# EffortlessMetrics/BitNet-rs

Measured on AMD Instinct MI355X. Metric: decode tokens/sec + I2_S matmul HBM GB/s (% roofline), bitnet-b1.58-2B-4T, higher is better.
Workload: dtype i8 MFMA on producer-quantised activations (QAct: 15-bit fixed point per element, one power-of-two scale per 16), exact integer partial sums, f32 accumulate / f32 elsewhere (f16 embedding table); 1 GPU; bitnet-b1.58-2B-4T I2_S BitNet32-F16 (ternary, one f16 scale per 32 weights), 1xMI355X, batch=1 decode, 128-token prompt; layers=30, prompt_len=128, parallelism=single GPU, launch=hipGraph replay per token, kv_cache=f32 (as the reference, T:1171-1202)

## Files before the change

bitnet-rs_amd/csrc/kernels_decode.hip:

```cpp
#include <cstdlib>

#include "common.hpp"

namespace bitnet_hip {

typedef _Float16 half8 __attribute__((ext_vector_type(8)));

__device__ __forceinline__ float wsum(float v) {
#pragma unroll
    for (int off = 32; off > 0; off >>= 1) v += __shfl_xor(v, off, 64);
    return v;
}
__device__ __forceinline__ float wmax(float v) {
#pragma unroll
    for (int off = 32; off > 0; off >>= 1) v = fmaxf(v, __shfl_xor(v, off, 64));
    return v;
}
__device__ __forceinline__ float bsum(float v, float *slot) {
    v = wsum(v);
    __syncthreads();
    if ((threadIdx.x & 63) == 0) slot[threadIdx.x >> 6] = v;
    __syncthreads();
    return (slot[0] + slot[1]) + (slot[2] + slot[3]);
}
__device__ __forceinline__ float bmax(float v, float *slot) {
    v = wmax(v);
    __syncthreads();
    if ((threadIdx.x & 63) == 0) slot[threadIdx.x >> 6] = v;
    __syncthreads();
    return fmaxf(fmaxf(slot[0], slot[1]), fmaxf(slot[2], slot[3]));
}

__global__ void k_embed_f16(const _Float16 *__restrict__ table, const int *__restrict__ tokens,
                            const int *__restrict__ offset_ptr, int n, int hidden, int vocab,
                            float *__restrict__ out) {
    const int per_row = hidden >> 3;
    const int gid = blockIdx.x * blockDim.x + threadIdx.x;
    if (gid >= n * per_row) return;
    const int t = gid / per_row, c = gid % per_row;
    int tok = tokens[t + (offset_ptr ? *offset_ptr : 0)];
    tok = tok < 0 ? 0 : (tok >= vocab ? vocab - 1 : tok);
    const half8 h = *reinterpret_cast<const half8 *>(table + (size_t)tok * hidden + 8 * c);
    float *o = out + (size_t)t * hidden + 8 * c;
#pragma unroll
    for (int i = 0; i < 8; ++i) o[i] = (float)h[i];
}

hipError_t launch_embed_f16(const void *table, const int *tokens, const int *offset_ptr, int n, int hidden,
                            int vocab, float *out, hipStream_t stream) {
    const int total = n * (hidden >> 3);
    hipLaunchKernelGGL(k_embed_f16, dim3((total + 255) / 256), dim3(256), 0, stream,
                       static_cast<const _Float16 *>(table), tokens, offset_ptr, n, hidden, vocab, out);
    return hipGetLastError();
}

template <bool RMS>
__global__ __launch_bounds__(256) void k_norm_rows(const float *__restrict__ x, const float *__restrict__ gamma,
                                                   float *__restrict__ out, int hidden, float eps) {
    __shared__ float slot[4];
    const float *xr = x + (size_t)blockIdx.x * hidden;
    float *orow = out + (size_t)blockIdx.x * hidden;
    float mean = 0.0f;
    if (!RMS) {
        float s = 0.0f;
        for (int i = threadIdx.x; i < hidden; i += 256) s += xr[i];
        mean = bsum(s, slot) / (float)hidden;
    }
    float ss = 0.0f;
    for (int i = threadIdx.x; i < hidden; i += 256) {
        const float d = xr[i] - mean;
        ss += d * d;
    }
    const float denom = sqrtf(bsum(ss, slot) / (float)hidden + eps);
    for (int i = threadIdx.x; i < hidden; i += 256) orow[i] = (xr[i] - mean) / denom * gamma[i];
}

hipError_t launch_norm_rows(const float *x, const float *gamma, float *out, int rows, int hidden, float eps,
                            bool rms, hipStream_t stream) {
    if (rows <= 0) return hipSuccess;
    if (rms)
        hipLaunchKernelGGL(k_norm_rows<true>, dim3(rows), dim3(256), 0, stream, x, gamma, out, hidden, eps);
    else
        hipLaunchKernelGGL(k_norm_rows<false>, dim3(rows), dim3(256), 0, stream, x, gamma, out, hidden, eps);
    return hipGetLastError();
}

constexpr int kLogitChunks = 16;

template <int NCH, int R, bool GUARD = false>
__global__ __launch_bounds__(256) void k_logits_f16(const _Float16 *__restrict__ table, const float *__restrict__ x,
                                                    const float *__restrict__ gamma, float eps, int hidden, int vocab,
                                                    float *__restrict__ logits, float *__restrict__ best_val,
                                                    int *__restrict__ best_idx) {
    extern __shared__ __attribute__((aligned(16))) float xs[];
    __shared__ float slot[4];
    __shared__ float wbv[4];
    __shared__ int wbi[4];
    const int tid = threadIdx.x, lane = tid & 63, wave = tid >> 6;
    float s = 0.0f;
    for (int i = tid; i < hidden; i += 256) s += x[i];
    const float mean = gamma ? bsum(s, slot) / (float)hidden : 0.0f;
    float ss = 0.0f;
    for (int i = tid; i < hidden; i += 256) {
        const float d = x[i] - mean;
        ss += d * d;
    }
    const float denom = gamma ? sqrtf(bsum(ss, slot) / (float)hidden + eps) : 1.0f;
    for (int i = tid; i < hidden; i += 256) xs[i] = gamma ? (x[i] - mean) / denom * gamma[i] : x[i];
    __syncthreads();
    const int nchunks = hidden >> 9;
    float xr[NCH][8];
#pragma unroll
    for (int c = 0; c < NCH; ++c)
#pragma unroll
        for (int i = 0; i < 8; ++i) xr[c][i] = (!GUARD || c < nchunks) ? xs[512 * c + 8 * lane + i] : 0.0f;
    float bv = -INFINITY;
    int bi = 0x7fffffff;
    const int total_waves = gridDim.x * 4;
    for (int row = (blockIdx.x * 4 + wave) * R; row < vocab; row += total_waves * R) {
        half8 w[R][NCH];
#pragma unroll
        for (int r = 0; r < R; ++r) {
            const _Float16 *e = table + (size_t)(row + r < vocab ? row + r : vocab - 1) * hidden + 8 * lane;
#pragma unroll
            for (int c = 0; c < NCH; ++c)
                w[r][c] = __builtin_nontemporal_load(reinterpret_cast<const half8 *>(e + 512 * ((!GUARD || c < nchunks) ? c : 0)));
        }
        float acc[R];
#pragma unroll
        for (int r = 0; r < R; ++r) {
            acc[r] = 0.0f;
#pragma unroll
            for (int c = 0; c < NCH; ++c)
#pragma unroll
                for (int i = 0; i < 8; ++i) acc[r] += xr[c][i] * (float)w[r][c][i];
        }
#pragma unroll
        for (int off = 32; off > 0; off >>= 1)
#pragma unroll
            for (int r = 0; r < R; ++r) acc[r] += __shfl_xor(acc[r], off, 64);
        if (lane == 0) {
#pragma unroll
            for (int r = 0; r < R; ++r)
                if (row + r < vocab) {
                    logits[row + r] = acc[r];
                    const float v = acc[r] != acc[r] ? -INFINITY : acc[r];
                    if (v > bv || (v == bv && row + r < bi)) {
                        bv = v;
                        bi = row + r;
                    }
                }
        }
    }
    if (lane == 0) {
        wbv[wave] = bv;
        wbi[wave] = bi;
    }
    __syncthreads();
    if (tid == 0) {
        for (int w2 = 1; w2 < 4; ++w2)
            if (wbv[w2] > bv || (wbv[w2] == bv && wbi[w2] < bi)) {
                bv = wbv[w2];
                bi = wbi[w2];
            }
        best_val[blockIdx.x] = bv;
        best_idx[blockIdx.x] = bi;
    }
}

__global__ __launch_bounds__(256) void k_argmax_final(const float *__restrict__ best_val, const int *__restrict__ best_idx,
                                                      int n, int *__restrict__ token_out, int *__restrict__ pos_ptr,
                                                      int *__restrict__ history, const int *__restrict__ n_forced) {
    __shared__ float sv[256];
    __shared__ int si[256];
    float bv = -INFINITY;
    int bi = 0x7fffffff;
    for (int i = threadIdx.x; i < n; i += 256) {
        const float v = best_val[i];
        const int idx = best_idx[i];
        if (v > bv || (v == bv && idx < bi)) {
            bv = v;
            bi = idx;
        }
    }
    sv[threadIdx.x] = bv;
    si[threadIdx.x] = bi;
    __syncthreads();
    for (int off = 128; off > 0; off >>= 1) {
        if ((int)threadIdx.x < off) {
            const float v = sv[threadIdx.x + off];
            const int idx = si[threadIdx.x + off];
            if (v > sv[threadIdx.x] || (v == sv[threadIdx.x] && idx < si[threadIdx.x])) {
                sv[threadIdx.x] = v;
                si[threadIdx.x] = idx;
            }
        }
        __syncthreads();
    }
    if (threadIdx.x == 0) {
        const int tok = si[0] == 0x7fffffff ? 0 : si[0];
        if (token_out) *token_out = tok;
        if (pos_ptr) {
            const int p = *pos_ptr;
            if (history && (!n_forced || p + 1 >= *n_forced)) history[p + 1] = tok;
            *pos_ptr = p + 1;
        }
    }
}

hipError_t launch_logits_f16(const void *table, const float *x, const float *gamma, float eps, int hidden, int vocab,
                             float *logits, float *best_val, int *best_idx, int n_wg, hipStream_t stream) {
    if (hidden % 512 != 0 || hidden > 512 * kLogitChunks) return hipErrorInvalidValue;
    void (*kfn)(const _Float16 *, const float *, const float *, float, int, int, float *, float *, int *) = nullptr;
    static const int rows = getenv("BITNET_HIP_LOGIT_ROWS") ? atoi(getenv("BITNET_HIP_LOGIT_ROWS")) : 3;
    switch (hidden / 512) {
        case 1: kfn = k_logits_f16<1, 4>; break;
        case 2: kfn = k_logits_f16<2, 4>; break;
        case 4: kfn = k_logits_f16<4, 4>; break;
        case 5: kfn = rows == 2 ? k_logits_f16<5, 2> : rows == 3 ? k_logits_f16<5, 3> : k_logits_f16<5, 4>; break;
        case 8: kfn = k_logits_f16<8, 2>; break;
        default: kfn = hidden / 512 <= 8 ? k_logits_f16<8, 2, true> : k_logits_f16<16, 1, true>; break;
    }
    hipLaunchKernelGGL(kfn, dim3(n_wg), dim3(256), (size_t)hidden * sizeof(float), stream, static_cast<const _Float16 *>(table), x, gamma,
                       eps, hidden, vocab, logits, best_val, best_idx);
    return hipGetLastError();
}

hipError_t launch_argmax_final(const float *best_val, const int *best_idx, int n, int *token_out, int *pos_ptr,
                               int *history, const int *n_forced, hipStream_t stream) {
    hipLaunchKernelGGL(k_argmax_final, dim3(1), dim3(256), 0, stream, best_val, best_idx, n, token_out, pos_ptr, history,
                       n_forced);
    return hipGetLastError();
}

__global__ void k_add(const float *__restrict__ a, const float *__restrict__ b, float *__restrict__ out, size_t n) {
    const size_t i = (size_t)blockIdx.x * blockDim.x + threadIdx.x;
    if (i < n) out[i] = a[i] + b[i];
}
hipError_t launch_add(const float *a, const float *b, float *out, size_t n, hipStream_t stream) {
    hipLaunchKernelGGL(k_add, dim3((unsigned)((n + 255) / 256)), dim3(256), 0, stream, a, b, out, n);
    return hipGetLastError();
}
__global__ void k_silu_mul(const float *__restrict__ gate, const float *__restrict__ up, float *__restrict__ out, size_t n, size_t tile) {
    const size_t i = (size_t)blockIdx.x * blockDim.x + threadIdx.x;
    if (i >= n) return;
    const size_t j = tile ? (i / tile) * 2 * tile + i % tile : i;
    const float g = gate[j], u = up[j];
    out[i] = g / (1.0f + expf(-g)) * u;
}
hipError_t launch_silu_mul(const float *gate, const float *up, float *out, size_t n, size_t tile, hipStream_t stream) {
    hipLaunchKernelGGL(k_silu_mul, dim3((unsigned)((n + 255) / 256)), dim3(256), 0, stream, gate, up, out, n, tile);
    return hipGetLastError();
}

__global__ void k_advance_pos(int *pos_ptr) {
    if (threadIdx.x == 0 && blockIdx.x == 0) *pos_ptr = *pos_ptr + 1;
}
hipError_t launch_advance_pos(int *pos_ptr, hipStream_t stream) {
    hipLaunchKernelGGL(k_advance_pos, dim3(1), dim3(64), 0, stream, pos_ptr);
    return hipGetLastError();
}

__global__ __launch_bounds__(256) void k_argmax_partial(const float *__restrict__ v, int n, float *__restrict__ best_val,
                                                        int *__restrict__ best_idx) {
    __shared__ float sv[256];
    __shared__ int si[256];
    float bv = -INFINITY;
    int bi = 0x7fffffff;
    for (int i = blockIdx.x * 256 + threadIdx.x; i < n; i += gridDim.x * 256) {
        const float a = v[i] != v[i] ? -INFINITY : v[i];
        if (a > bv || (a == bv && i < bi)) {
            bv = a;
            bi = i;
        }
    }
    sv[threadIdx.x] = bv;
    si[threadIdx.x] = bi;
    __syncthreads();
    for (int off = 128; off > 0; off >>= 1) {
        if ((int)threadIdx.x < off) {
            const float a = sv[threadIdx.x + off];
            const int idx = si[threadIdx.x + off];
            if (a > sv[threadIdx.x] || (a == sv[threadIdx.x] && idx < si[threadIdx.x])) {
                sv[threadIdx.x] = a;
                si[threadIdx.x] = idx;
            }
        }
        __syncthreads();
    }
    if (threadIdx.x == 0) {
        best_val[blockIdx.x] = sv[0];
        best_idx[blockIdx.x] = si[0];
    }
}

hipError_t launch_argmax(const float *v, int n, float *best_val, int *best_idx, int n_wg, int *token_out,
                         hipStream_t stream) {
    hipLaunchKernelGGL(k_argmax_partial, dim3(n_wg), dim3(256), 0, stream, v, n, best_val, best_idx);
    hipLaunchKernelGGL(k_argmax_final, dim3(1), dim3(256), 0, stream, best_val, best_idx, n_wg, token_out, nullptr, nullptr, nullptr);
    return hipGetLastError();
}

__global__ __launch_bounds__(512) void k_stream_read(const uint4 *__restrict__ buf, size_t n_vec, unsigned *sink) {
    const size_t stride = (size_t)gridDim.x * 512 * 8;
    unsigned acc = 0;
    for (size_t i = ((size_t)blockIdx.x * 8) * 512 + threadIdx.x; i < n_vec; i += stride) {
        uint4 v[8];
#pragma unroll
        for (int j = 0; j < 8; ++j) {
            const size_t idx = i + (size_t)j * 512;
            const unsigned *p = reinterpret_cast<const unsigned *>(buf + (idx < n_vec ? idx : i));
            v[j].x = __builtin_nontemporal_load(p);
            v[j].y = __builtin_nontemporal_load(p + 1);
            v[j].z = __builtin_nontemporal_load(p + 2);
            v[j].w = __builtin_nontemporal_load(p + 3);
        }
#pragma unroll
        for (int j = 0; j < 8; ++j) acc ^= v[j].x ^ v[j].y ^ v[j].z ^ v[j].w;
    }
    if (acc == 0x9e3779b9u) *sink = acc;
}

hipError_t launch_stream_read(const void *buf, size_t bytes, unsigned *sink, hipStream_t stream) {
    const size_t n_vec = bytes / 16;
    size_t grid = div_ceil(n_vec, (size_t)512 * 8 * 4);
    if (grid < 256) grid = 256;
    if (grid > 65535u * 16u) grid = 65535u * 16u;
    hipLaunchKernelGGL(k_stream_read, dim3((unsigned)grid), dim3(512), 0, stream, static_cast<const uint4 *>(buf), n_vec, sink);
    return hipGetLastError();
}

}
```

bitnet-rs_amd/host/decoder.hpp:

```cpp
#pragma once

#include <cstddef>
#include <cstdint>
#include <string>
#include <vector>

#include "bitnet_hip.h"

extern "C" {
typedef int (*bitnet_host_allgather_fn)(void *ctx, const void *send_dev, void *recv_dev, size_t bytes_per_rank, void *stream);
}

namespace bitnet_host {

struct Config {
    int hidden = 2560, n_layers = 30, n_heads = 20, n_kv_heads = 5, head_dim = 128;
    int ffn = 6912, vocab = 128256, max_pos = 4096;
    float eps = 1e-5f;
    float rope_theta = 10000.f;
};

struct LayerWeightsQk256 {
    const float *attn_norm, *ffn_norm;
    const uint8_t *q, *k, *v, *o, *gate, *up, *down;
};
struct LayerWeightsI2s {
    const float *attn_norm, *ffn_norm;
    const uint8_t *w[7];
    const float *scales[7];
    size_t block_size;
};

struct ProjSpec {
    bool qk256 = true;
    const uint8_t *bytes = nullptr;
    size_t len = 0;
    const float *scales = nullptr;
    size_t n_scales = 0, block = 32;
    int8_t code_map[4] = {-2, -1, 0, 1};
};

class Decoder {
  public:
    explicit Decoder(const Config &cfg);
    ~Decoder();
    Decoder(const Decoder &) = delete;
    Decoder &operator=(const Decoder &) = delete;

    const Config &config() const { return c_; }
    const std::string &error() const { return err_; }
    bool dead() const { return dead_; }
    void set_error(const std::string &e) { err_ = e; }

    int set_layer_qk256(int layer, const LayerWeightsQk256 &w);
    int set_layer_i2s(int layer, const LayerWeightsI2s &w);
    int set_layer_specs(int layer, const float *attn_norm, const float *ffn_norm, const ProjSpec p[7]);
    int set_globals(const uint16_t *embed_f16, const float *final_norm);

    int reset();
    int set_sampling(const bitnet_hip_sampling_config *cfg);
    int sampling_draws(uint64_t *out);
    int feed(const int32_t *tokens, int n);
    int run(int n, bool with_logits, bool use_graph, float *elapsed_ms);
    int run_reference(int n, bool with_logits);
    int set_act_mode(int mode);
    int set_kv_f16(bool on);
    bool kv_f16() const { return kv_f16_; }
    bool qact_path() const;
    int prefill(int n, bool with_logits, int digits, float *elapsed_ms);
    int prefill_sharded(int n, int rank, int world, bitnet_host_allgather_fn gather, void *gather_ctx, bool with_logits, int digits,
                        bool wire_f16, float *elapsed_ms);
    int finish_prefill(int n, const float *last_row, bool with_logits);
    int score(int n, int digits, float *nll_out, int32_t *argmax_out, float *logits_out, int logits_rows, float *elapsed_ms);
    bool chain_applies(int digits) const;
    bool handover16_applies(int digits) const;
    bool hybrid_applies(size_t n_rows) const;
    int last_prefill_path() const { return last_prefill_path_; }
    int saturation_fallbacks() const { return saturation_fallbacks_; }
    int fp6_flag(int digits);
    int ensure_chain_buffers(size_t N);
    int prefill_chain_layers(size_t N);
    bool qb32_applies(int digits, size_t n_rows);
    int prefill_qb32_layers(size_t N);
    void set_phase_timing(bool on) { sp_timing_ = on; }
    void phase_times(float out[4]) const {
        for (int i = 0; i < 4; ++i) out[i] = sp_phase_us_[i];
    }
    void layer_objects(int layer, uint64_t handles[4], void *ptrs[4]) const;
    void global_objects(void *ptrs[7]) const;
    int position();
    int history(int32_t *out, int n);
    int last_logits(float *out);
    int last_hidden(float *out);
    int trace_step(const char *dir, bool with_logits);
    int probe_gateup(int reps, float *us_per_launch, double *bytes_per_launch);
    int probe_kernel(int kind, int reps, float *us_per_launch, double *bytes_per_launch);
    size_t weight_bytes() const { return weight_bytes_; }
    void *stream() const { return stream_; }

  private:
    int fail(const char *what);
    int fail_arg(const char *what);
    bool dead_ = false;
    struct Tracer;
    int step_launches(bool with_logits, int form, Tracer *tr = nullptr);
    int step_launches_reference(bool with_logits);
    int ensure_graph(bool with_logits, int form);
  public:
    int prepare_graphs(bool with_logits);
  private:
    int form_at(int pos) const;
    bool merge_ok_ = false;

    Config c_;
    std::string err_;
    void *stream_ = nullptr;
    struct Layer {
        float *attn_norm = nullptr, *ffn_norm = nullptr;
        bitnet_hip_weights_t qkv = 0, o = 0, gateup = 0, down = 0;
        float *kcache = nullptr, *vcache = nullptr;
        bool q_ok = false;
    };
    int attn_launch(Layer &L, int form, float *out, void *qout);
    void release_layer(Layer &L);
    void drop_graphs();
    int pick_token(void *stream);
    int adopt_projections(Layer &L, bitnet_hip_weights_t h[7]);
    std::vector<Layer> layers_;
    void *embed_ = nullptr;
    float *final_norm_ = nullptr;
    float *rope_sin_ = nullptr, *rope_cos_ = nullptr;
    float *x_ = nullptr, *x2_ = nullptr, *qkv_ = nullptr, *att_ = nullptr, *h_ = nullptr, *logits_ = nullptr;
    void *qa_x_ = nullptr, *qa_x2_ = nullptr, *qa_att_ = nullptr, *qa_h_ = nullptr;
    double *st_x_ = nullptr, *st_x2_ = nullptr;
    int act_mode_ = 1;
    bool kv_f16_ = false;
    std::string trace_dir_;
    float *ref_n_ = nullptr, *ref_gu_ = nullptr, *ref_t_ = nullptr;
    void *scratch_ = nullptr;
    float *attn_scratch_ = nullptr;
    int32_t *pos_ = nullptr, *n_forced_ = nullptr, *history_ = nullptr, *token_ = nullptr;
    bitnet_hip_sampler *sampler_ = nullptr;
    bool sampling_ = false;
    int host_forced_ = 0;
    int sp_cap_ = 0, sp_ctx_ = 0;
    void *sp_kv_send_ = nullptr, *sp_kv_all_ = nullptr;
    void *comm_stream_ = nullptr, *sp_ev_pack_ = nullptr, *sp_ev_gather_ = nullptr;
    int32_t *sp_block_pos_ = nullptr, *sp_tokens_ = nullptr;
    bool sp_timing_ = false;
    std::vector<void *> sp_tev_;
    float sp_phase_us_[4] = {0.f, 0.f, 0.f, 0.f};
    int pf_cap_ = 0;
    float *pf_x_ = nullptr, *pf_qkv_ = nullptr, *pf_att_ = nullptr, *pf_h_ = nullptr;
    void *pf_gemm_ws_ = nullptr, *pf_attn_ws_ = nullptr;
    int pfc_cap_ = 0;
    void *pf_xh_ = nullptr, *pf_atth_ = nullptr, *pf_hh_ = nullptr;
    float *pf_stats_ = nullptr;
    void *pf_qb_ = nullptr;
    int pf_qb_cap_ = 0;
    bool force_scaled_ = false;
    int saturation_fallbacks_ = 0;
    int sc_cap_ = 0, sc_logits_cap_ = 0;
    int32_t *sc_tgt_ = nullptr, *sc_am_ = nullptr;
    float *sc_nll_ = nullptr, *sc_logits_ = nullptr;
    void *sc_ws_ = nullptr;
    size_t sc_ws_bytes_ = 0;
    int last_prefill_path_ = 0;
    int prefill_qb32_ = -1;
    int prefill_fp6_ = -1;
    int prefill_chain_ = -1;
    size_t pf_gemm_ws_bytes_ = 0, pf_attn_ws_bytes_ = 0;
    size_t weight_bytes_ = 0;
    static constexpr int kGraphs = 6;
    void *graph_exec_[kGraphs] = {};
    void *graph_[kGraphs] = {};
    int logits_wgs_ = 512;
};

}

extern "C" {
typedef struct bitnet_host_config {
    int32_t hidden, n_layers, n_heads, n_kv_heads, head_dim, ffn, vocab, max_pos;
    float eps, rope_theta;
} bitnet_host_config;
void *bitnet_host_create(const bitnet_host_config *cfg);
void bitnet_host_destroy(void *d);
const char *bitnet_host_error(void *d);
int bitnet_host_set_layer_qk256(void *d, int layer, const float *attn_norm, const float *ffn_norm,
                                const uint8_t *q, const uint8_t *k, const uint8_t *v, const uint8_t *o,
                                const uint8_t *gate, const uint8_t *up, const uint8_t *down);
int bitnet_host_set_layer_i2s(void *d, int layer, const float *attn_norm, const float *ffn_norm,
                              const uint8_t *const *w7, const float *const *scales7, size_t block_size);
int bitnet_host_set_globals(void *d, const uint16_t *embed_f16, const float *final_norm);
int bitnet_host_reset(void *d);
int bitnet_host_set_sampling(void *d, const bitnet_hip_sampling_config *cfg);
int bitnet_host_sampling_draws(void *d, uint64_t *out);
int bitnet_host_feed(void *d, const int32_t *tokens, int n);
int bitnet_host_run(void *d, int n, int with_logits, int use_graph, float *elapsed_ms);
int bitnet_host_run_reference(void *d, int n, int with_logits);
int bitnet_host_prepare_graphs(void *d, int with_logits);
int bitnet_host_set_act_mode(void *d, int mode);
int bitnet_host_set_kv_f16(void *d, int on);
int bitnet_host_act_mode(void *d);
int bitnet_host_prefill(void *d, int n, int with_logits, int digits, float *elapsed_ms);
int bitnet_host_finish_prefill(void *d, int n, const float *last_row, int with_logits);
int bitnet_host_score(void *d, int n, int digits, float *nll_out, int32_t *argmax_out, float *logits_out, int logits_rows, float *elapsed_ms);
int bitnet_host_set_phase_timing(void *d, int on);
int bitnet_host_phase_times(void *d, float out[4]);
int bitnet_host_prefill_sharded(void *d, int n, int rank, int world, bitnet_host_allgather_fn gather, void *gather_ctx, int with_logits,
                                int digits, int wire_f16, float *elapsed_ms);
int bitnet_host_rccl_allgather(void *nccl_comm, const void *send_dev, void *recv_dev, size_t bytes_per_rank, void *stream);
void bitnet_host_layer_objects(void *d, int layer, uint64_t *handles4, void **ptrs4);
void bitnet_host_global_objects(void *d, void **ptrs7);
int bitnet_host_position(void *d);
int bitnet_host_history(void *d, int32_t *out, int n);
int bitnet_host_last_logits(void *d, float *out);
int bitnet_host_last_hidden(void *d, float *out);
int bitnet_host_trace_step(void *d, const char *dir, int with_logits);
int bitnet_host_blake3_hex(const void *data, size_t len, char *out65);
int bitnet_host_probe_gateup(void *d, int reps, float *us_per_launch, double *bytes_per_launch);
int bitnet_host_probe_kernel(void *d, int kind, int reps, float *us_per_launch, double *bytes_per_launch);
uint64_t bitnet_host_weight_bytes(void *d);
}
```

Measured before the change: 1211 tokens/s.

## Double-buffer logits row loads and prefetch first rows before final norm

The f16 logits kernel now issues the first batch of embedding-row loads before computing the final RMS/layer norm, so the norm reduction overlaps with HBM latency. The row loop is software-pipelined with two register buffers, so the next rows are requested before the current ones are reduced. x and gamma are read into registers once rather than re-read from global memory. The default rows per wave rises from 3 to 4 and the logits grid from 512 to 1002 workgroups. This raises register pressure and may lower occupancy, and the prefetch loads past vocab are clamped to the last row.

```diff
diff --git a/bitnet-rs_amd/csrc/kernels_decode.hip b/bitnet-rs_amd/csrc/kernels_decode.hip
--- a/bitnet-rs_amd/csrc/kernels_decode.hip
+++ b/bitnet-rs_amd/csrc/kernels_decode.hip
@@ -87,6 +87,49 @@
 
 constexpr int kLogitChunks = 16;
 
+template <int NCH, int R, bool GUARD>
+__device__ __forceinline__ void logit_rows_request(half8 (&w)[R][NCH], const _Float16 *__restrict__ table, int row, int vocab, int hidden,
+                                                   int nchunks, int lane) {
+#pragma unroll
+    for (int r = 0; r < R; ++r) {
+        const bool in = row + r < vocab;
+        const _Float16 *e = table + (size_t)(in ? row + r : vocab - 1) * hidden + (in ? 8 * lane : 0);
+#pragma unroll
+        for (int c = 0; c < NCH; ++c)
+            w[r][c] = __builtin_nontemporal_load(reinterpret_cast<const half8 *>(e + (in ? 512 * ((!GUARD || c < nchunks) ? c : 0) : 0)));
+    }
+}
+
+template <int NCH, int R>
+__device__ __forceinline__ void logit_rows_finish(const half8 (&w)[R][NCH], const float (&xr)[NCH][8], int row, int vocab, int lane,
+                                                  float *__restrict__ logits, float &bv, int &bi) {
+    float acc[R];
+#pragma unroll
+    for (int r = 0; r < R; ++r) {
+        acc[r] = 0.0f;
+#pragma unroll
+        for (int c = 0; c < NCH; ++c)
+#pragma unroll
+            for (int i = 0; i < 8; ++i) acc[r] += xr[c][i] * (float)w[r][c][i];
+    }
+#pragma unroll
+    for (int off = 32; off > 0; off >>= 1)
+#pragma unroll
+        for (int r = 0; r < R; ++r) acc[r] += __shfl_xor(acc[r], off, 64);
+    if (lane == 0) {
+#pragma unroll
+        for (int r = 0; r < R; ++r)
+            if (row + r < vocab) {
+                logits[row + r] = acc[r];
+                const float v = acc[r] != acc[r] ? -INFINITY : acc[r];
+                if (v > bv || (v == bv && row + r < bi)) {
+                    bv = v;
+                    bi = row + r;
+                }
+            }
+    }
+}
+
 template <int NCH, int R, bool GUARD = false>
 __global__ __launch_bounds__(256) void k_logits_f16(const _Float16 *__restrict__ table, const float *__restrict__ x,
                                                     const float *__restrict__ gamma, float eps, int hidden, int vocab,
@@ -96,19 +139,45 @@
     __shared__ float slot[4];
     __shared__ float wbv[4];
     __shared__ int wbi[4];
-    const int tid = threadIdx.x, lane = tid & 63, wave = tid >> 6;
+    const int tid = threadIdx.x, lane = tid & 63;
+    const int wave = __builtin_amdgcn_readfirstlane(tid >> 6);
+    const int nchunks = hidden >> 9;
+    const int stride = gridDim.x * 4 * R;
+    int row = (blockIdx.x * 4 + wave) * R;
+    constexpr int XV = 2 * NCH;
+    float xv[XV], gv[XV] = {};
+#pragma unroll
+    for (int j = 0; j < XV; ++j) {
+        const int i = tid + 256 * j;
+        xv[j] = x[(!GUARD || i < hidden) ? i : tid];
+    }
+    if (gamma) {
+#pragma unroll
+        for (int j = 0; j < XV; ++j) {
+            const int i = tid + 256 * j;
+            gv[j] = gamma[(!GUARD || i < hidden) ? i : tid];
+        }
+    }
+    half8 wa[R][NCH], wb[R][NCH];
+    logit_rows_request<NCH, R, GUARD>(wa, table, row, vocab, hidden, nchunks, lane);
+    __builtin_amdgcn_sched_barrier(0);
     float s = 0.0f;
-    for (int i = tid; i < hidden; i += 256) s += x[i];
+#pragma unroll
+    for (int j = 0; j < XV; ++j)
+        if (!GUARD || tid + 256 * j < hidden) s += xv[j];
     const float mean = gamma ? bsum(s, slot) / (float)hidden : 0.0f;
     float ss = 0.0f;
-    for (int i = tid; i < hidden; i += 256) {
-        const float d = x[i] - mean;
-        ss += d * d;
-    }
+#pragma unroll
+    for (int j = 0; j < XV; ++j)
+        if (!GUARD || tid + 256 * j < hidden) {
+            const float d = xv[j] - mean;
+            ss += d * d;
+        }
     const float denom = gamma ? sqrtf(bsum(ss, slot) / (float)hidden + eps) : 1.0f;
-    for (int i = tid; i < hidden; i += 256) xs[i] = gamma ? (x[i] - mean) / denom * gamma[i] : x[i];
-    __syncthreads();
-    const int nchunks = hidden >> 9;
+#pragma unroll
+    for (int j = 0; j < XV; ++j)
+        if (!GUARD || tid + 256 * j < hidden) xs[tid + 256 * j] = gamma ? (xv[j] - mean) / denom * gv[j] : xv[j];
+    __syncthreads();
     float xr[NCH][8];
 #pragma unroll
     for (int c = 0; c < NCH; ++c)
@@ -116,41 +185,13 @@
         for (int i = 0; i < 8; ++i) xr[c][i] = (!GUARD || c < nchunks) ? xs[512 * c + 8 * lane + i] : 0.0f;
     float bv = -INFINITY;
     int bi = 0x7fffffff;
-    const int total_waves = gridDim.x * 4;
-    for (int row = (blockIdx.x * 4 + wave) * R; row < vocab; row += total_waves * R) {
-        half8 w[R][NCH];
-#pragma unroll
-        for (int r = 0; r < R; ++r) {
-            const _Float16 *e = table + (size_t)(row + r < vocab ? row + r : vocab - 1) * hidden + 8 * lane;
-#pragma unroll
-            for (int c = 0; c < NCH; ++c)
-                w[r][c] = __builtin_nontemporal_load(reinterpret_cast<const half8 *>(e + 512 * ((!GUARD || c < nchunks) ? c : 0)));
-        }
-        float acc[R];
-#pragma unroll
-        for (int r = 0; r < R; ++r) {
-            acc[r] = 0.0f;
-#pragma unroll
-            for (int c = 0; c < NCH; ++c)
-#pragma unroll
-                for (int i = 0; i < 8; ++i) acc[r] += xr[c][i] * (float)w[r][c][i];
-        }
-#pragma unroll
-        for (int off = 32; off > 0; off >>= 1)
-#pragma unroll
-            for (int r = 0; r < R; ++r) acc[r] += __shfl_xor(acc[r], off, 64);
-        if (lane == 0) {
-#pragma unroll
-            for (int r = 0; r < R; ++r)
-                if (row + r < vocab) {
-                    logits[row + r] = acc[r];
-                    const float v = acc[r] != acc[r] ? -INFINITY : acc[r];
-                    if (v > bv || (v == bv && row + r < bi)) {
-                        bv = v;
-                        bi = row + r;
-                    }
-                }
-        }
+    for (; row < vocab; row += 2 * stride) {
+        logit_rows_request<NCH, R, GUARD>(wb, table, row + stride, vocab, hidden, nchunks, lane);
+        __builtin_amdgcn_sched_barrier(0);
+        logit_rows_finish<NCH, R>(wa, xr, row, vocab, lane, logits, bv, bi);
+        logit_rows_request<NCH, R, GUARD>(wa, table, row + 2 * stride, vocab, hidden, nchunks, lane);
+        __builtin_amdgcn_sched_barrier(0);
+        logit_rows_finish<NCH, R>(wb, xr, row + stride, vocab, lane, logits, bv, bi);
     }
     if (lane == 0) {
         wbv[wave] = bv;
@@ -212,7 +253,7 @@
                              float *logits, float *best_val, int *best_idx, int n_wg, hipStream_t stream) {
     if (hidden % 512 != 0 || hidden > 512 * kLogitChunks) return hipErrorInvalidValue;
     void (*kfn)(const _Float16 *, const float *, const float *, float, int, int, float *, float *, int *) = nullptr;
-    static const int rows = getenv("BITNET_HIP_LOGIT_ROWS") ? atoi(getenv("BITNET_HIP_LOGIT_ROWS")) : 3;
+    static const int rows = getenv("BITNET_HIP_LOGIT_ROWS") ? atoi(getenv("BITNET_HIP_LOGIT_ROWS")) : 4;
     switch (hidden / 512) {
         case 1: kfn = k_logits_f16<1, 4>; break;
         case 2: kfn = k_logits_f16<2, 4>; break;
diff --git a/bitnet-rs_amd/host/decoder.hpp b/bitnet-rs_amd/host/decoder.hpp
--- a/bitnet-rs_amd/host/decoder.hpp
+++ b/bitnet-rs_amd/host/decoder.hpp
@@ -174,7 +174,7 @@
     static constexpr int kGraphs = 6;
     void *graph_exec_[kGraphs] = {};
     void *graph_[kGraphs] = {};
-    int logits_wgs_ = 512;
+    int logits_wgs_ = 1002;
 };
 
 }
```

Result: no change. 1216 tokens/s, median of 3 (+0.4%).
